# RomanBresson/KAGNN

Measured on AMD Instinct MI355X. Metric: edges/sec KAN-GIN fwd+bwd, hidden=64 grid=5, 1M-node synthetic; HBM % peak, higher is better.
Workload: dtype f32 (fp16 hi/lo split operands, fp32 accumulate)

## Files before the change

kagnn_amd/csrc/aggregate.hip:

```cpp
#include "common.h"
#include "host.h"

namespace kagnn {


__device__ __forceinline__ float4 ld4(const float* p) { return *reinterpret_cast<const float4*>(p); }
__device__ __forceinline__ void fma4(float4& a, float w, const float4& v) {
    a.x = fmaf(w, v.x, a.x); a.y = fmaf(w, v.y, a.y); a.z = fmaf(w, v.z, a.z); a.w = fmaf(w, v.w, a.w);
}

__device__ __forceinline__ float edge_w(const AggArgs& a, int e, int j, long i) {
    float w = a.ew ? a.ew[e] : 1.0f;
    if (a.in_scale) w *= a.in_scale[j];
    if (a.skip_self && j == (int)i) w = 0.0f;
    return w;
}

__device__ __forceinline__ void stats_products(const AggArgs& a, long row, int c4, const float4& o, float4& pa, float4& pb) {
    const float4 y = ld4(a.st_y + row * a.st_ldy + c4), m = ld4(a.st_mean + c4), q = ld4(a.st_rstd + c4);
    pa = o;
    pb = make_float4(o.x * ((y.x - m.x) * q.x), o.y * ((y.y - m.y) * q.y), o.z * ((y.z - m.z) * q.z), o.w * ((y.w - m.w) * q.w));
}

template <int LPR, bool STATS = false>
__global__ __launch_bounds__(256) void agg_rows_v4_kernel(AggArgs a) {
    const unsigned wg = (blockIdx.x & 7) * (gridDim.x >> 3) + (blockIdx.x >> 3);
    const long gid = (wg * 256L + threadIdx.x) / LPR;
    const int c4 = (threadIdx.x % LPR) * 4;
    const bool live = gid < a.N && c4 < a.F;
    if (!STATS && !live) return;
    float4 pa = make_float4(0.f, 0.f, 0.f, 0.f), pb = pa;
    if (live) {
        const int s = a.rowptr[gid], t = a.rowptr[gid + 1];
        const bool hub = (t - s) > a.hub_threshold;
        float4 acc = ld4(a.x + gid * a.ldx + c4);
        const float sw = a.self_scale * (a.in_scale ? a.in_scale[gid] : 1.0f);
        acc.x *= sw; acc.y *= sw; acc.z *= sw; acc.w *= sw;
        if (!hub) {
            int e = s;
            for (; e + 4 <= t; e += 4) {
                const int j0 = a.col[e], j1 = a.col[e + 1], j2 = a.col[e + 2], j3 = a.col[e + 3];
                const float4 v0 = ld4(a.x + (long)j0 * a.ldx + c4);
                const float4 v1 = ld4(a.x + (long)j1 * a.ldx + c4);
                const float4 v2 = ld4(a.x + (long)j2 * a.ldx + c4);
                const float4 v3 = ld4(a.x + (long)j3 * a.ldx + c4);
                fma4(acc, edge_w(a, e, j0, gid), v0);
                fma4(acc, edge_w(a, e + 1, j1, gid), v1);
                fma4(acc, edge_w(a, e + 2, j2, gid), v2);
                fma4(acc, edge_w(a, e + 3, j3, gid), v3);
            }
            for (; e < t; ++e) {
                const int j = a.col[e];
                fma4(acc, edge_w(a, e, j, gid), ld4(a.x + (long)j * a.ldx + c4));
            }
        }
        const float os = a.out_scale ? a.out_scale[gid] : 1.0f;
        float4 b = make_float4(0.f, 0.f, 0.f, 0.f);
        if (a.bias) b = ld4(a.bias + c4);
        float4 o = make_float4(fmaf(os, acc.x, b.x), fmaf(os, acc.y, b.y), fmaf(os, acc.z, b.z), fmaf(os, acc.w, b.w));
        if (a.col_scale) {
            const float4 cs = ld4(a.col_scale + c4), ch = ld4(a.col_shift + c4);
            const float cnt = (float)(t - s) + a.self_scale;
            o.x = fmaf(cs.x, o.x, cnt * ch.x); o.y = fmaf(cs.y, o.y, cnt * ch.y);
            o.z = fmaf(cs.z, o.z, cnt * ch.z); o.w = fmaf(cs.w, o.w, cnt * ch.w);
        }
        if (a.addend && !hub) {
            const float4 d = ld4(a.addend + gid * a.lda + c4);
            o.x += d.x; o.y += d.y; o.z += d.z; o.w += d.w;
        }
        *reinterpret_cast<float4*>(a.out + gid * a.ldo + c4) = o;
        if (STATS && !hub) stats_products(a, gid, c4, o, pa, pb);
    }
    if constexpr (STATS) {
        __shared__ float4 s_a[256], s_b[256];
        s_a[threadIdx.x] = pa; s_b[threadIdx.x] = pb;
        __syncthreads();
        if (threadIdx.x < LPR && c4 < a.F && wg * 256L < a.N * LPR) {
            constexpr int R = 256 / LPR;
#pragma unroll 4
            for (int k = 1; k < R; ++k) {
                const float4 u = s_a[k * LPR + threadIdx.x], v = s_b[k * LPR + threadIdx.x];
                pa.x += u.x; pa.y += u.y; pa.z += u.z; pa.w += u.w;
                pb.x += v.x; pb.y += v.y; pb.z += v.z; pb.w += v.w;
            }
            *reinterpret_cast<float4*>(a.st_partial + (wg * 2L + 0) * a.F + c4) = pa;
            *reinterpret_cast<float4*>(a.st_partial + (wg * 2L + 1) * a.F + c4) = pb;
        }
    }
}

template <int LPR>
__global__ __launch_bounds__(256) void agg_rows_ep_kernel(AggArgs a) {
    constexpr int EP = 16 / LPR;
    const long gid = (blockIdx.x * 256L + threadIdx.x) >> 4;
    const int l16 = threadIdx.x & 15, cg = l16 % LPR, eg = l16 / LPR;
    const int c4 = cg * 4;
    const bool live = gid < a.N && c4 < a.F;
    const long row = min(gid, a.N - 1);
    const int cc = live ? c4 : 0;
    const int s = a.rowptr[row], t = a.rowptr[row + 1];
    const bool hub = (t - s) > a.hub_threshold;
    float4 acc = make_float4(0.f, 0.f, 0.f, 0.f);
    if (!hub) {
        int e = s + eg;
        for (; e + EP < t; e += 2 * EP) {
            const int j0 = a.col[e], j1 = a.col[e + EP];
            const float4 v0 = ld4(a.x + (long)j0 * a.ldx + cc);
            const float4 v1 = ld4(a.x + (long)j1 * a.ldx + cc);
            fma4(acc, edge_w(a, e, j0, row), v0);
            fma4(acc, edge_w(a, e + EP, j1, row), v1);
        }
        if (e < t) {
            const int j = a.col[e];
            fma4(acc, edge_w(a, e, j, row), ld4(a.x + (long)j * a.ldx + cc));
        }
    }
#pragma unroll
    for (int o = LPR; o < 16; o <<= 1) {
        acc.x += __shfl_xor(acc.x, o); acc.y += __shfl_xor(acc.y, o);
        acc.z += __shfl_xor(acc.z, o); acc.w += __shfl_xor(acc.w, o);
    }
    if (live && eg == 0) {
        const float sw = a.self_scale * (a.in_scale ? a.in_scale[row] : 1.0f);
        const float4 xs = ld4(a.x + row * a.ldx + c4);
        const float os = a.out_scale ? a.out_scale[row] : 1.0f;
        float4 b = make_float4(0.f, 0.f, 0.f, 0.f);
        if (a.bias) b = ld4(a.bias + c4);
        float4 o = make_float4(fmaf(os, fmaf(sw, xs.x, acc.x), b.x), fmaf(os, fmaf(sw, xs.y, acc.y), b.y),
                               fmaf(os, fmaf(sw, xs.z, acc.z), b.z), fmaf(os, fmaf(sw, xs.w, acc.w), b.w));
        if (a.col_scale) {
            const float4 cs = ld4(a.col_scale + c4), ch = ld4(a.col_shift + c4);
            const float cnt = (float)(t - s) + a.self_scale;
            o.x = fmaf(cs.x, o.x, cnt * ch.x); o.y = fmaf(cs.y, o.y, cnt * ch.y);
            o.z = fmaf(cs.z, o.z, cnt * ch.z); o.w = fmaf(cs.w, o.w, cnt * ch.w);
        }
        if (a.addend && !hub) {
            const float4 d = ld4(a.addend + row * a.lda + c4);
            o.x += d.x; o.y += d.y; o.z += d.z; o.w += d.w;
        }
        *reinterpret_cast<float4*>(a.out + row * a.ldo + c4) = o;
    }
}

template <int LPR>
__global__ __launch_bounds__(256) void agg_hub_v4_kernel(AggArgs a, const int* __restrict__ seg,
                                                         float* __restrict__ part, int ldp) {
    __shared__ float4 s_part[256];
    const int row = seg[3 * blockIdx.x], e0 = seg[3 * blockIdx.x + 1], e1 = seg[3 * blockIdx.x + 2];
    constexpr int G = 256 / LPR;
    const int g = threadIdx.x / LPR, lg = threadIdx.x % LPR, c4 = lg * 4;
    float4 acc = make_float4(0.f, 0.f, 0.f, 0.f);
    if (c4 < a.F) {
        int e = e0 + g;
        for (; e + 3 * G < e1; e += 4 * G) {
            const int j0 = a.col[e], j1 = a.col[e + G], j2 = a.col[e + 2 * G], j3 = a.col[e + 3 * G];
            const float4 v0 = ld4(a.x + (long)j0 * a.ldx + c4);
            const float4 v1 = ld4(a.x + (long)j1 * a.ldx + c4);
            const float4 v2 = ld4(a.x + (long)j2 * a.ldx + c4);
            const float4 v3 = ld4(a.x + (long)j3 * a.ldx + c4);
            fma4(acc, edge_w(a, e, j0, row), v0);
            fma4(acc, edge_w(a, e + G, j1, row), v1);
            fma4(acc, edge_w(a, e + 2 * G, j2, row), v2);
            fma4(acc, edge_w(a, e + 3 * G, j3, row), v3);
        }
        for (; e < e1; e += G) {
            const int j = a.col[e];
            fma4(acc, edge_w(a, e, j, row), ld4(a.x + (long)j * a.ldx + c4));
        }
    }
    s_part[threadIdx.x] = acc;
    __syncthreads();
    if (g == 0 && c4 < a.F) {
#pragma unroll 8
// ... 229 lines not shown
        }
        for (; b < b1; ++b) a += partial[b * per + k];
    }
    s_part[sub][e] = a;
    __syncthreads();
    if (sub == 0 && k < per) {
        float t = s_part[0][e];
#pragma unroll
        for (int q = 1; q < 8; ++q) t += s_part[q][e];
        g_table[k] = t;
    }
}

int embedding_fwd(const int64_t* idx, long stride, long N, const float* table, int V, int F, float* out, long ldo, int accumulate,
                  hipStream_t st) {
    if (N == 0) return KAGNN_OK;
    embedding_fwd_kernel<<<cdiv(N, 4), 256, 0, st>>>(idx, stride, N, table, V, F, out, ldo, accumulate);
    KAGNN_LAUNCH_CHECK();
    return KAGNN_OK;
}

size_t embedding_bwd_ws_bytes(long N, int V, int F) { return (size_t)cdiv(max(N, 1L), kEmbRows) * V * F * sizeof(float); }

int embedding_bwd(const int64_t* idx, long stride, long N, const float* g, long ldg, int V, int F, float* g_table, float* ws,
                  size_t ws_bytes, hipStream_t st) {
    if (V == 0) return KAGNN_OK;
    if (V > 512) return fail(KAGNN_ERR_UNSUPPORTED, "%s: tables of at most 512 rows (the categorical encoders of the graph-level models)", "embedding_bwd");
    if (ws_bytes < embedding_bwd_ws_bytes(N, V, F)) return fail(KAGNN_ERR_ARG, "%s: workspace too small", "embedding_bwd");
    const size_t tbl = (size_t)V * 64 * sizeof(float);
    const int waves = 4 * tbl <= 64 * 1024 ? 4 : 2 * tbl <= 128 * 1024 ? 2 : 1;
    const int nb = cdiv(max(N, 1L), (long)kEmbRows);
    const size_t lds = waves * tbl;
    if (lds > 64 * 1024) {
        static unsigned long long configured = 0;
        if (auto first_use_ = first_use_on_this_device(configured)) {
            KAGNN_HIP(hipFuncSetAttribute((const void*)embedding_bwd_partial_kernel<1>, hipFuncAttributeMaxDynamicSharedMemorySize, 128 * 1024 + 1024));
            KAGNN_HIP(hipFuncSetAttribute((const void*)embedding_bwd_partial_kernel<2>, hipFuncAttributeMaxDynamicSharedMemorySize, 128 * 1024 + 1024));
        }
    }
    const dim3 grid((unsigned)nb, (unsigned)cdiv(F, 64));
    if (waves == 4) embedding_bwd_partial_kernel<4><<<grid, 256, lds, st>>>(idx, stride, N, g, ldg, V, F, ws);
    else if (waves == 2) embedding_bwd_partial_kernel<2><<<grid, 128, lds, st>>>(idx, stride, N, g, ldg, V, F, ws);
    else embedding_bwd_partial_kernel<1><<<grid, 64, lds, st>>>(idx, stride, N, g, ldg, V, F, ws);
    KAGNN_LAUNCH_CHECK();
    embedding_bwd_reduce_kernel<<<cdiv((long)V * F, 32), 256, 0, st>>>(ws, nb, V, F, g_table);
    KAGNN_LAUNCH_CHECK();
    return KAGNN_OK;
}

static bool vec4_ok(const AggArgs& a) {
    auto al = [](const void* p) { return (reinterpret_cast<uintptr_t>(p) & 15) == 0; };
    return a.F % 4 == 0 && a.F <= 256 && a.ldx % 4 == 0 && a.ldo % 4 == 0 && al(a.x) && al(a.out) &&
           (!a.bias || al(a.bias)) && (!a.addend || (al(a.addend) && a.lda % 4 == 0)) &&
           (!a.col_scale || (al(a.col_scale) && al(a.col_shift)));
}

size_t aggregate_ws_bytes(long num_hub_seg, int F) { return (size_t)num_hub_seg * (size_t)((F + 3) & ~3) * sizeof(float); }

int aggregate_hub_rows(const AggArgs& a, const int* hub_seg, long num_hub_seg, float* ws, size_t ws_bytes, hipStream_t st) {
    if (num_hub_seg <= 0) return KAGNN_OK;
    const int ldp = (a.F + 3) & ~3;
    if ((size_t)num_hub_seg * ldp * sizeof(float) > ws_bytes) return fail(KAGNN_ERR_ARG, "%s: workspace too small", "aggregate_hub_rows");
#define HUBS(LPR)                                                                                   \
    {                                                                                               \
        agg_hub_v4_kernel<LPR><<<(unsigned)num_hub_seg, 256, 0, st>>>(a, hub_seg, ws, ldp);         \
        KAGNN_LAUNCH_CHECK();                                                                       \
        agg_hub_merge_kernel<LPR><<<(unsigned)num_hub_seg, 256, 0, st>>>(a, hub_seg, num_hub_seg, ws, ldp); \
        KAGNN_LAUNCH_CHECK();                                                                       \
    }
    if (a.F <= 4) HUBS(1) else if (a.F <= 8) HUBS(2) else if (a.F <= 16) HUBS(4) else if (a.F <= 32) HUBS(8)
    else if (a.F <= 64) HUBS(16) else if (a.F <= 128) HUBS(32) else HUBS(64)
#undef HUBS
    return KAGNN_OK;
}

static int stats_lpr(int F) { return F <= 32 ? 8 : F <= 64 ? 16 : F <= 128 ? 32 : 64; }
bool aggregate_stats_ok(const AggArgs& a) {
    auto al = [](const void* p) { return (reinterpret_cast<uintptr_t>(p) & 15) == 0; };
    return vec4_ok(a) && a.F > 16 && a.st_y && a.st_mean && a.st_rstd && a.st_partial && a.st_ldy % 4 == 0 && al(a.st_y) &&
           al(a.st_mean) && al(a.st_rstd) && al(a.st_partial);
}
long aggregate_stats_rows(long N, int F, long num_hub_seg) { return (long)cdiv(N * stats_lpr(F), 256) + (num_hub_seg > 0 ? num_hub_seg : 0); }

int aggregate_sum(const AggArgs& a, const int* hub_seg, long num_hub_seg, float* ws, size_t ws_bytes, hipStream_t st) {
    if (a.N == 0) return KAGNN_OK;
    const bool stats = a.st_partial != nullptr;
    if (stats && !aggregate_stats_ok(a)) return fail(KAGNN_ERR_UNSUPPORTED, "%s: column statistics need 16-byte aligned fp32 rows of 17..256 columns", "aggregate_sum");
    if (!vec4_ok(a)) {
        AggArgs b = a;
        b.hub_threshold = 0x7fffffff;
        dim3 grid((unsigned)a.N, cdiv(a.F, 256));
        agg_rows_generic_kernel<<<grid, 256, 0, st>>>(b);
        KAGNN_LAUNCH_CHECK();
        return KAGNN_OK;
    }
    AggArgs b = a;
    if (num_hub_seg == 0 || hub_seg == nullptr) b.hub_threshold = 0x7fffffff;
    const int ldp = (a.F + 3) & ~3;
    if (b.hub_threshold != 0x7fffffff && (ws == nullptr || ws_bytes < aggregate_ws_bytes(num_hub_seg, a.F)))
        return fail(KAGNN_ERR_ARG, "%s: workspace too small for the hub segments (see kagnn_aggregate_workspace_bytes)", "aggregate_sum");
#define HUBS(LPR, ST)                                                                               \
    if (b.hub_threshold != 0x7fffffff) {                                                            \
        agg_hub_v4_kernel<LPR><<<(unsigned)num_hub_seg, 256, 0, st>>>(b, hub_seg, ws, ldp);         \
        KAGNN_LAUNCH_CHECK();                                                                       \
        agg_hub_merge_kernel<LPR, ST><<<(unsigned)num_hub_seg, 256, 0, st>>>(b, hub_seg, num_hub_seg, ws, ldp, (long)cdiv(a.N * LPR, 256)); \
        KAGNN_LAUNCH_CHECK();                                                                       \
    }
#define AGG_ROWS_GRID(threads) (cdiv(cdiv((threads), 256), 8) * 8)
#define ROWS(LPR)                                                                     \
    {                                                                                 \
        if (stats) {                                                                  \
            agg_rows_v4_kernel<LPR, true><<<AGG_ROWS_GRID(a.N * LPR), 256, 0, st>>>(b);   \
            KAGNN_LAUNCH_CHECK();                                                     \
            HUBS(LPR, true)                                                           \
        } else {                                                                      \
            agg_rows_v4_kernel<LPR><<<AGG_ROWS_GRID(a.N * LPR), 256, 0, st>>>(b);       \
            KAGNN_LAUNCH_CHECK();                                                     \
            HUBS(LPR, false)                                                          \
        }                                                                             \
    }
#define ROWS_EP(LPR)                                                                  \
    {                                                                                 \
        agg_rows_ep_kernel<LPR><<<cdiv(a.N * 16, 256), 256, 0, st>>>(b);              \
        KAGNN_LAUNCH_CHECK();                                                         \
        HUBS(LPR, false)                                                              \
    }
    if (a.F <= 4) ROWS_EP(1) else if (a.F <= 8) ROWS_EP(2) else if (a.F <= 16) ROWS_EP(4) else if (a.F <= 32) ROWS(8)
    else if (a.F <= 64) ROWS(16)
    else if (a.F <= 128) ROWS(32) else ROWS(64)
#undef ROWS
#undef AGG_ROWS_GRID
#undef ROWS_EP
#undef HUBS
    return KAGNN_OK;
}

int gcn_deg_inv_sqrt(const int* rowptr, const int* col, long N, float* dis, hipStream_t st) {
    if (N == 0) return KAGNN_OK;
    gcn_deg_kernel<<<cdiv(N, 256), 256, 0, st>>>(rowptr, col, N, dis);
    KAGNN_LAUNCH_CHECK();
    return KAGNN_OK;
}

int gine_fwd(const float* x, long ldx, const float* ea, long lde, float* out, long ldo,
             const int* rowptr, const int* col, const int* perm, long N, int F, float self_scale,
             hipStream_t st) {
    if (N == 0) return KAGNN_OK;
    gine_fwd_kernel<<<cdiv(N, 4), 256, 0, st>>>(x, ldx, ea, lde, out, ldo, rowptr, col, perm, N, F, self_scale);
    KAGNN_LAUNCH_CHECK();
    return KAGNN_OK;
}

int gine_bwd(const float* x, long ldx, const float* ea, long lde, const float* gout, long ldg,
             float* gx, long ldgx, float* gea, long ldge, const int* rowptr, const int* col,
             const int* perm, long N, int F, float self_scale, hipStream_t st, int gea_accumulate) {
    if (N == 0) return KAGNN_OK;
    gine_bwd_kernel<<<cdiv(N, 4), 256, 0, st>>>(x, ldx, ea, lde, gout, ldg, gx, ldgx, gea, ldge, rowptr, col, perm, N, F, self_scale, gea_accumulate);
    KAGNN_LAUNCH_CHECK();
    return KAGNN_OK;
}

int segment_pool(const float* x, long ldx, float* out, long ldo, const int* seg, long B, int F,
                 int mean, hipStream_t st) {
    if (B == 0) return KAGNN_OK;
    segment_pool_kernel<<<cdiv(B, 4), 256, 0, st>>>(x, ldx, out, ldo, seg, B, F, mean);
    KAGNN_LAUNCH_CHECK();
    return KAGNN_OK;
}

int segment_bcast(const float* g, long ldg, float* gx, long ldgx, const int* seg, long B, int F,
                  int mean, hipStream_t st) {
    if (B == 0) return KAGNN_OK;
    segment_bcast_kernel<<<cdiv(B, 4), 256, 0, st>>>(g, ldg, gx, ldgx, seg, B, F, mean);
    KAGNN_LAUNCH_CHECK();
    return KAGNN_OK;
}

}
```

kagnn_amd/csrc/common.h:

```cpp
#pragma once
#include <hip/hip_runtime.h>
#include <stdint.h>
#include <stdio.h>
#include <string.h>
#include "../../include/kagnn_hip.h"

namespace kagnn {

extern thread_local char g_err[512];
extern thread_local bool g_half_products;
inline int fail(int code, const char* fmt, const char* a = "", long b = 0, long c = 0) {
    snprintf(g_err, sizeof(g_err), fmt, a, b, c);
    return code;
}
#define KAGNN_CHECK_ARG_AS(fn, cond, msg)                                                \
    do {                                                                                 \
        if (!(cond)) return kagnn::fail(KAGNN_ERR_ARG, "%s: argument check failed: " msg, fn); \
    } while (0)
#define KAGNN_CHECK_ARG(cond, msg) KAGNN_CHECK_ARG_AS(__func__, cond, msg)
#define KAGNN_HIP(...)                                                                   \
    do {                                                                                 \
        hipError_t e_ = (__VA_ARGS__);                                                   \
        if (e_ != hipSuccess) {                                                          \
            snprintf(kagnn::g_err, sizeof(kagnn::g_err), "%s: HIP error at line %d -> %s", __func__, __LINE__, \
// ... 116 lines not shown
    const bool finite = fabsf(x) <= 3.4028234e38f;
    const float nanv = __builtin_nanf("");
#pragma unroll
    for (int r = 0; r <= K; ++r) {
        N[r] = finite ? (inside ? n[r] : 0.0f) : nanv;
        if (DERIV) dN[r] = finite ? (inside ? dN[r] : 0.0f) : nanv;
    }
    return m;
}

template <int K, bool DERIV>
__device__ __forceinline__ int bspline_generic(float x, const float* __restrict__ t ,
                                               int nknots, float (&N)[K + 1], float (&dN)[K + 1]) {
    int cnt = 0;
    for (int j = 0; j < nknots; ++j) cnt += (x >= t[j]) ? 1 : 0;
    const bool inside = cnt >= 1 && cnt < nknots;
    const int m = min(max(cnt - 1, 0), nknots - 2);
    float w[2 * K + 2];
#pragma unroll
    for (int q = 0; q < 2 * K + 2; ++q) w[q] = t[min(max(m - K + q, 0), nknots - 1)];
    float n[K + 1], prev[K + 1];
    n[0] = 1.0f;
#pragma unroll
    for (int r = 1; r <= K; ++r) n[r] = 0.0f;
#pragma unroll
    for (int p = 1; p <= K; ++p) {
#pragma unroll
        for (int r = 0; r <= K; ++r) prev[r] = n[r];
#pragma unroll
        for (int r = 0; r <= p; ++r) {
            const int q0 = K - p + r;
            const float a = (r >= 1) ? (x - w[q0]) / (w[q0 + p] - w[q0]) * prev[r - 1] : 0.0f;
            const float b = (r <= p - 1) ? (w[q0 + p + 1] - x) / (w[q0 + p + 1] - w[q0 + 1]) * prev[r] : 0.0f;
            n[r] = a + b;
        }
        if (DERIV && p == K) {
#pragma unroll
            for (int r = 0; r <= K; ++r) {
                const float lo = (r >= 1) ? prev[r - 1] / (w[r + K] - w[r]) : 0.0f;
                const float hi = (r <= K - 1) ? prev[r] / (w[r + K + 1] - w[r + 1]) : 0.0f;
                dN[r] = (float)K * (lo - hi);
            }
        }
    }
    const bool finite = fabsf(x) <= 3.4028234e38f;
    const float nanv = __builtin_nanf("");
#pragma unroll
    for (int r = 0; r <= K; ++r) {
        N[r] = finite ? (inside ? n[r] : 0.0f) : nanv;
        if (DERIV) dN[r] = finite ? (inside ? dN[r] : 0.0f) : nanv;
    }
    return m;
}

template <int K, bool DERIV, bool PF>
__device__ __forceinline__ int eval_basis(float x, const float* s_knots, const SplineGeom& g,
                                          const float* __restrict__ knots_g, int f, float (&N)[K + 1],
                                          float (&dN)[K + 1]) {
    if constexpr (PF) return bspline_generic<K, DERIV>(x, knots_g + (long)f * g.nknots, g.nknots, N, dN);
    else return bspline_local<K, DERIV>(x, s_knots, g, N, dN);
}

template <int K>
__device__ __forceinline__ float pick_basis(const float (&N)[K + 1], int m, int c) {
    const int d = c - (m - K);
    float a = 0.0f;
#pragma unroll
    for (int r = 0; r <= K; ++r) a = (d == r) ? N[r] : a;
    return a;
}

struct AggArgs {
    const float* x; long ldx;
    float* out; long ldo;
    const int* rowptr; const int* col; const float* ew;
    long N; int F;
    float self_scale;
    const float* in_scale; const float* out_scale; const float* bias;
    int skip_self; int hub_threshold;
    const float* addend; long lda;
    const float* col_scale = nullptr; const float* col_shift = nullptr;
    const float* st_y = nullptr; long st_ldy = 0; const float* st_mean = nullptr; const float* st_rstd = nullptr;
    float* st_partial = nullptr;
};

struct EdgeGradArgs {
    const float* x; long ldx;
    const float* gout; long ldg;
    const int* rowptr; const int* col; const int* perm;
    long N; long E; int F;
    const float* in_scale; const float* out_scale;
    int skip_self; int hub_threshold;
    float* out;
};

struct BnBack {
    const float* y; long ldy;
    const float* tab; int ldt;
    float* gy_out; long ldo;
};
#ifdef __HIPCC__
__device__ __forceinline__ float bn_bwd_value(float g, float y, float m, float A, float B, float C) {
    return __builtin_fmaf(A, g, __builtin_fmaf(B, __fsub_rn(y, m), C));
}
__device__ __forceinline__ void bn_bwd_consts(float q , float gamma, float sum_g, float sum_gxhat, float inv_n, float& A,
                                              float& B, float& C) {
    const float k = __fmul_rn(q, gamma);
    A = k;
    B = -__fmul_rn(__fmul_rn(k, q), __fmul_rn(sum_gxhat, inv_n));
    C = -__fmul_rn(k, __fmul_rn(sum_g, inv_n));
}
#endif

inline hipStream_t as_stream(void* s) { return reinterpret_cast<hipStream_t>(s); }

}
```

kagnn_amd/csrc/fused_calls.hip:

```cpp
#include "host.h"

using namespace kagnn;

namespace {
struct GraphSide {
    const int32_t* rowptr; const int32_t* col; const int32_t* hub_seg; int64_t num_hub_seg; int32_t hub_threshold; float self_scale;
};
struct KanChain {
    int64_t N; int32_t L; const int32_t* widths;
    const float* const* bw; const float* const* sw; const float* const* sc;
    const float* const* acts; const void* const* pack_fwd; const void* const* pack_dx;
    const float* knots; int32_t G, K, mode;
};
struct LayerIn {
    const void* x; int32_t x_dtype; int64_t ldx; const float* in_col_scale; const float* in_col_shift; float* col_mean; float* col_m2;
};
struct LayerGrads {
    const float* gy; int64_t ldgy; void* gx; int32_t gx_dtype; int64_t ldgx; int32_t bf16_gather; const float* gx_addend; int64_t ld_addend;
    float* const* g_bw; float* const* g_sw; float* const* g_sc;
};

struct GineStage {
    const float* x; int64_t ldx; const float* ea; int64_t lde; const int32_t* perm;
    float* g_ea; int64_t ldge;
    int accumulate_g_ea = 0;
    int prepacked = 0;
};
struct BnStage { const float* y; int64_t ldy; const float* weight; const float* mean; const float* rstd; float* g_weight; float* g_bias; };
struct StatsOut { const float* y; int64_t ldy; const float* mean; const float* rstd; float* sums; };
struct DwPiece { unsigned char* base; DwDefer* defer; };

struct LayerLayout {
    size_t fwd_hub_bytes, fwd_scratch, fwd_scratch_bytes, fwd_fix, fwd_fix_bytes, fwd_total;
    size_t bwd_hub_bytes, dw, dw_bytes, g[2], bwd_total;
    size_t bn, bn_ws_bytes, bn_tab, bn_bytes, stats, stats_bytes, bwd_total_all;
    size_t dw_piece[8], dw_piece_bytes[8], dw_pieces_bytes;
    int wmax;
};

void layer_layout_optional(LayerLayout& y, int64_t N, int out, int f0, int64_t num_hub_seg_t) {
    y.bn = y.bwd_total;
    y.bn_ws_bytes = out ? bn_ws_bytes(N, out) : 0;
    y.bn_tab = y.bn + al256z(y.bn_ws_bytes);
    y.bn_bytes = out ? al256z(y.bn_ws_bytes) + al256z(4 * (size_t)((out + 63) & ~63) * sizeof(float)) : 0;
    y.stats = y.bn + y.bn_bytes;
    y.stats_bytes = f0 ? al256z(bn_stats_fold_bytes(aggregate_stats_rows(N, f0, num_hub_seg_t), f0)) : 0;
    y.bwd_total_all = y.stats + y.stats_bytes;
}

int layer_layout(int64_t N, int32_t L, const int32_t* widths, int32_t G, int32_t K, int32_t mode, int64_t num_hub_seg,
                 int64_t num_hub_seg_t, LayerLayout& y) {
    static const char fn[] = "kagnn_gin_kan_layer_workspace_bytes";
    size_t fw = 0, dw = 0;
    y.wmax = 0;
    for (int l = 0; l < L; ++l) {
        int rc = check_kan_dims(fn, widths[l], widths[l + 1], G, K, mode);
        if (rc) return rc;
        size_t b = 0;
        rc = (l == L - 1 ? kagnn_kan_fwd_moments_workspace_bytes : kagnn_kan_fwd_workspace_bytes)(N, widths[l], widths[l + 1], G, K, mode, &b);
        if (rc) return rc;
        fw = b > fw ? b : fw;
        rc = kagnn_kan_bwd_weight_workspace_bytes(N, widths[l], widths[l + 1], G, K, mode, &b); if (rc) return rc;
        dw = b > dw ? b : dw;
        y.dw_piece_bytes[l] = al256z(b);
        y.wmax = widths[l] > y.wmax ? widths[l] : y.wmax;
    }
    y.dw_pieces_bytes = 0;
    for (int l = L - 1; l >= 0; --l) { y.dw_piece[l] = y.dw_pieces_bytes; y.dw_pieces_bytes += y.dw_piece_bytes[l]; }
    y.fwd_hub_bytes = al256z(aggregate_bf16_ws_bytes(num_hub_seg, widths[0]));
    y.fwd_scratch = y.fwd_hub_bytes;
    y.fwd_fix = y.fwd_scratch + al256z(fw);
    y.fwd_total = y.fwd_fix + al256z(widths[0] <= 32 ? kan_sparse_fwd_agg_ws_bytes(num_hub_seg, widths[0], widths[1]) : 0) + 256;
    y.fwd_scratch_bytes = y.fwd_total - y.fwd_scratch;
    y.fwd_fix_bytes = y.fwd_total - y.fwd_fix;
    y.bwd_hub_bytes = al256z(aggregate_bf16_ws_bytes(num_hub_seg_t, widths[0]));
    y.dw = y.bwd_hub_bytes;
    y.dw_bytes = al256z(dw);
    const size_t g_bytes = al256z((size_t)N * y.wmax * sizeof(float));
    y.g[0] = y.dw + y.dw_bytes;
    y.g[1] = y.g[0] + g_bytes;
    y.bwd_total = y.g[1] + g_bytes + 256;
    layer_layout_optional(y, N, 0, 0, 0);
    return KAGNN_OK;
}

int layer_fwd_impl(const GraphSide& gr, const KanChain& c, const LayerIn& in, const GineStage* gine, void* workspace,
                   size_t workspace_bytes, void* stream, const char* fn) {
    (void)fn;
    const int64_t N = c.N;
    const int32_t L = c.L, G = c.G, K = c.K, mode = c.mode;
    const int32_t* widths = c.widths;
    float* const* acts = const_cast<float* const*>(c.acts);
    void* const* pack_fwd = const_cast<void* const*>(c.pack_fwd);
    void* const* pack_dx = const_cast<void* const*>(c.pack_dx);
    KAGNN_CHECK_ARG(N >= 0 && L >= 1 && L <= 8 && widths && c.bw && c.sw && acts && pack_fwd && pack_dx, "bad argument");
    KAGNN_CHECK_ARG((in.in_col_scale == nullptr) == (in.in_col_shift == nullptr), "in_col_scale and in_col_shift must both be given or both be null");
    KAGNN_CHECK_ARG(!in.in_col_scale || in.x_dtype == KAGNN_DTYPE_F32, "the column affine of the gathered matrix needs fp32 rows");
    KAGNN_CHECK_ARG((in.col_mean == nullptr) == (in.col_m2 == nullptr), "col_mean and col_m2 must both be given or both be null");
    LayerLayout lay;
    int rc = layer_layout(N, L, widths, G, K, mode, gr.num_hub_seg, 0, lay);
    if (rc) return rc;
    KAGNN_CHECK_ARG(workspace && workspace_bytes >= lay.fwd_total, "workspace too small (kagnn_gin_kan_layer_workspace_bytes)");
    if (N == 0) return KAGNN_OK;
    unsigned char* ws = static_cast<unsigned char*>(workspace);
    const char* fuse_e = getenv("KAGNN_FUSE_AGG");
    const bool fuse_env = fuse_e != nullptr && atoi(fuse_e) != 0;
    const bool fuse = fuse_env && !gine && !in.in_col_scale && in.x_dtype == KAGNN_DTYPE_F32 && mode == KAGNN_PREC_SPLIT && !(L == 1 && in.col_mean) &&
                      use_sparse_fwd(widths[0], widths[1], G, K, mode) &&
                      kan_sparse_fwd_agg_ok(static_cast<const float*>(in.x), in.ldx, N, widths[0], widths[1], G, K);
    if (gine)
        rc = kagnn_aggregate_gine(static_cast<const float*>(in.x), in.ldx, gine->ea, gine->lde, acts[0], widths[0], gr.rowptr, gr.col, gine->perm, N,
                                  widths[0], gr.self_scale, stream);
    else if (fuse)
        rc = KAGNN_OK;
    else if (in.x_dtype == KAGNN_DTYPE_BF16)
        rc = kagnn_aggregate_sum_bf16(in.x, in.ldx, acts[0], widths[0], KAGNN_DTYPE_F32, gr.rowptr, gr.col, nullptr, N, widths[0], gr.self_scale,
                                      nullptr, nullptr, nullptr, 0, gr.hub_seg, gr.num_hub_seg, gr.hub_threshold, ws, lay.fwd_hub_bytes, stream);
    else if (in.in_col_scale)
        rc = kagnn_aggregate_sum_affine(static_cast<const float*>(in.x), in.ldx, acts[0], widths[0], gr.rowptr, gr.col, N, widths[0], gr.self_scale,
                                        in.in_col_scale, in.in_col_shift, gr.hub_seg, gr.num_hub_seg, gr.hub_threshold, nullptr, 0, ws,
                                        lay.fwd_hub_bytes, stream);
    else
        rc = kagnn_aggregate_sum(static_cast<const float*>(in.x), in.ldx, acts[0], widths[0], gr.rowptr, gr.col, nullptr, N, widths[0],
                                 gr.self_scale, nullptr, nullptr, nullptr, 0, gr.hub_seg, gr.num_hub_seg, gr.hub_threshold, ws, lay.fwd_hub_bytes,
                                 stream);
    if (rc) return rc;
    const bool prepacked = gine && gine->prepacked;
    bool batched = L >= 2 && !prepacked;
    int in_[8], out_[8];
    for (int l = 0; l < L; ++l) {
        in_[l] = widths[l]; out_[l] = widths[l + 1];
        batched = batched && use_split_dx(in_[l], out_[l], G, K, mode) && use_sparse_fwd(in_[l], out_[l], G, K, mode) &&
                  kan_fused_pack_ok(in_[l], out_[l], G + K);
    }
    if (batched) {
        rc = kagnn_kan_pack_batch(L, c.bw, c.sw, c.sc, in_, out_, G, K, mode, pack_fwd, pack_dx, stream);
        if (rc) return rc;
    } else if (!prepacked) {
        for (int l = 0; l < L; ++l) {
            rc = kagnn_kan_pack(c.bw[l], c.sw[l], c.sc ? c.sc[l] : nullptr, in_[l], out_[l], G, K, mode, pack_fwd[l], pack_dx[l], stream);
            if (rc) return rc;
        }
    }
    for (int l = 0; l < L; ++l) {
        if (l == 0 && fuse) {
            KAGNN_STAGE_AS("kagnn_kan_linear_fwd+aggregate_sum (one kernel)", stream);
            rc = kan_sparse_fwd_agg(static_cast<const float*>(in.x), in.ldx, N, gr.rowptr, gr.col, gr.hub_seg, gr.num_hub_seg, gr.hub_threshold,
                                    gr.self_scale, c.knots, in_[0], out_[0], G, K, pack_fwd[0], acts[0], in_[0], acts[1], out_[0],
                                    ws + lay.fwd_fix, lay.fwd_fix_bytes, as_stream(stream));
            if (rc) return rc;
            continue;
        }
        if (l == L - 1 && in.col_mean)
            rc = kagnn_kan_linear_fwd_moments(acts[l], in_[l], N, c.knots, in_[l], out_[l], G, K, mode, pack_fwd[l], acts[l + 1],
                                              out_[l], in.col_mean, in.col_m2, ws + lay.fwd_scratch, lay.fwd_scratch_bytes, stream);
        else
            rc = kagnn_kan_linear_fwd(acts[l], in_[l], N, c.knots, in_[l], out_[l], G, K, mode, pack_fwd[l], acts[l + 1], out_[l],
                                      ws + lay.fwd_scratch, lay.fwd_scratch_bytes, stream);
        if (rc) return rc;
    }
    return KAGNN_OK;
}

int layer_bwd_impl(const GraphSide& gr, const KanChain& c, const LayerGrads& io, const BnStage* bn, const float* bn_sums_in,
                   const StatsOut* so, const GineStage* gine, const DwPiece* piece, void* workspace, size_t workspace_bytes, void* stream,
                   const char* fn) {
    const int64_t N = c.N;
    const int32_t L = c.L, G = c.G, K = c.K, mode = c.mode;
    const int32_t* widths = c.widths;
    const float* const* acts = c.acts;
    void* const gx = io.gx;
    KAGNN_CHECK_ARG(N >= 0 && L >= 1 && L <= 8 && widths && c.sw && acts && c.pack_dx && io.g_sw, "bad argument");
    KAGNN_CHECK_ARG(!io.gx_addend || (gx && io.gx_dtype == KAGNN_DTYPE_F32 && !io.bf16_gather && io.ld_addend >= widths[0]),
                    "gx_addend needs an fp32 gx and fp32 gather operands");
    LayerLayout lay;
    int rc = layer_layout(N, L, widths, G, K, mode, 0, gr.num_hub_seg, lay);
    if (rc) return rc;
    layer_layout_optional(lay, N, bn ? widths[L] : 0, so ? widths[0] : 0, gr.num_hub_seg);
    KAGNN_CHECK_ARG(!so || (so->y && so->mean && so->rstd && so->sums && so->ldy >= widths[0] && gx && io.gx_dtype == KAGNN_DTYPE_F32 && !io.bf16_gather),
                    "the previous norm's statistics need its input, mean, rstd and an fp32 gx");
    KAGNN_CHECK_ARG(!bn_sums_in || bn, "bn_sums belongs to the BatchNorm stage");
    if (!(workspace && workspace_bytes >= lay.bwd_total_all))
        return fail(KAGNN_ERR_ARG, bn ? "%s: workspace too small (kagnn_gin_kan_layer_workspace_bytes + kagnn_gin_kan_layer_bwd_bn_workspace_bytes)"
                                      : "%s: workspace too small (kagnn_gin_kan_layer_workspace_bytes)", fn);
    if (N == 0) return KAGNN_OK;
    unsigned char* ws = static_cast<unsigned char*>(workspace);
    const int wmax = lay.wmax;
    unsigned char* gbuf[2] = {ws + lay.g[0], ws + lay.g[1]};
    auto dw = [&](int l, const float* g, long ldg) {
        unsigned char* area = piece ? piece->base + lay.dw_piece[l] : ws + lay.dw;
        const size_t bytes = piece ? lay.dw_piece_bytes[l] : lay.dw_bytes;
        return kan_linear_bwd_weight(acts[l], widths[l], nullptr, g, ldg, N, c.knots, widths[l], widths[l + 1], G, K, mode, c.sw[l],
                                     c.sc ? c.sc[l] : nullptr, io.g_bw ? io.g_bw[l] : nullptr, io.g_sw[l], io.g_sc ? io.g_sc[l] : nullptr,
                                     area, bytes, stream, piece ? piece->defer : nullptr);
    };
    const float* g = io.gy;
    long ldg = io.ldgy;
    int cur = 0;
    bool gh0_bf16 = false;
    bool bn_in_dx = false;
    BnBack bnb{};
    if (bn) {
        const int out = widths[L], ldt = (out + 63) & ~63;
        KAGNN_CHECK_ARG(bn->y && bn->mean && bn->rstd && bn->ldy >= out && N >= 2, "bad BatchNorm stage");
        unsigned char* bws = ws + lay.bn;
        float* tab = reinterpret_cast<float*>(ws + lay.bn_tab);
        bnb = BnBack{bn->y, (long)bn->ldy, tab, ldt, reinterpret_cast<float*>(gbuf[1]), (long)out};
        const int in = widths[L - 1];
        bn_in_dx = mode == KAGNN_PREC_SPLIT && use_split_dx(in, out, G, K, mode) && out <= wmax && !(L == 1 && (gx == nullptr || io.bf16_gather)) &&
                   fits32(N, ldg) && kan_split_dx_bn_ok(ldg, in, out, G, K, bnb, g);
        if (bn_in_dx && bn_sums_in) {
            KAGNN_STAGE_AS("kagnn_batchnorm_bwd statistics given (in ..._layer_bwd_bn)", stream);
            rc = bn_bwd_stats_given(bn_sums_in, N, out, bn->weight, bn->mean, bn->rstd, bn->g_weight, bn->g_bias, tab, ldt, as_stream(stream));
            if (rc) return rc;
        } else if (bn_in_dx) {
            KAGNN_STAGE_AS("kagnn_batchnorm_bwd statistics (in ..._layer_bwd_bn)", stream);
            rc = bn_bwd_stats(bn->y, bn->ldy, g, ldg, N, out, bn->weight, bn->mean, bn->rstd, bn->g_weight, bn->g_bias, tab, ldt, bws,
                              lay.bn_ws_bytes, as_stream(stream));
            if (rc) return rc;
        } else {
            if (out > wmax) return fail(KAGNN_ERR_UNSUPPORTED, "%s: a BatchNorm stage wider than every layer input is not covered", fn);
            KAGNN_STAGE_AS("kagnn_batchnorm_bwd", stream);
            rc = bn_bwd(bn->y, bn->ldy, g, ldg, N, out, bn->weight, bn->mean, bn->rstd, 1, 0.0f, 0ULL, reinterpret_cast<float*>(gbuf[1]), out,
                        bn->g_weight, bn->g_bias, bws, lay.bn_ws_bytes, as_stream(stream));
            if (rc) return rc;
            g = reinterpret_cast<const float*>(gbuf[1]); ldg = out;
        }
    }
    for (int l = L - 1; l >= 0; --l) {
        const int in = widths[l], out = widths[l + 1];
        const bool fused_bn = bn_in_dx && l == L - 1;
        if (fused_bn) {
            {
                KAGNN_STAGE_AS("kagnn_kan_linear_bwd_input", stream);
                rc = kan_split_dx_bn(acts[l], in, g, ldg, N, c.knots, in, out, G, K, c.pack_dx[l], reinterpret_cast<float*>(gbuf[0]), in, bnb,
                                     as_stream(stream));
            }
            if (rc) return rc;
            rc = dw(l, bnb.gy_out, bnb.ldo);
            if (rc) return rc;
            if (l == 0 && gx == nullptr) break;
            g = reinterpret_cast<const float*>(gbuf[0]); ldg = in; cur = 1;
            continue;
        }
        rc = dw(l, g, ldg);
        if (rc) return rc;
        if (l == 0 && gx == nullptr) break;
        const bool b16 = l == 0 && io.bf16_gather && mode == KAGNN_PREC_SPLIT && K == 3 && G + K <= 8 && out <= 128 && in % 8 == 0 &&
                         in <= 512  &&
                         use_split_dx(in, out, G, K, mode);
        rc = kagnn_kan_linear_bwd_input(acts[l], in, g, ldg, N, c.knots, in, out, G, K, mode, c.pack_dx[l], gbuf[cur], in,
                                        b16 ? KAGNN_DTYPE_BF16 : KAGNN_DTYPE_F32, stream);
        if (rc) return rc;
        g = reinterpret_cast<const float*>(gbuf[cur]); ldg = in; cur ^= 1;
        gh0_bf16 = b16;
    }
    if (gx == nullptr) return KAGNN_OK;
    const int f0 = widths[0];
    if (gine)
        return gine_bwd(gine->x, gine->ldx, gine->ea, gine->lde, g, ldg, static_cast<float*>(gx), io.ldgx, gine->g_ea, gine->ldge,
                        gr.rowptr, gr.col, gine->perm, N, f0, gr.self_scale, as_stream(stream), gine->accumulate_g_ea);
    if (gh0_bf16 || io.gx_dtype == KAGNN_DTYPE_BF16) {
        const void* src = g;
        if (!gh0_bf16) {
            rc = kagnn_rows_to_bf16(g, ldg, gbuf[cur], f0, N, f0, stream);
            if (rc) return rc;
            src = gbuf[cur];
        }
        return kagnn_aggregate_sum_bf16(src, f0, gx, io.ldgx, io.gx_dtype, gr.rowptr, gr.col, nullptr, N, f0, gr.self_scale, nullptr, nullptr,
                                        nullptr, 0, gr.hub_seg, gr.num_hub_seg, gr.hub_threshold, ws, lay.bwd_hub_bytes, stream);
    }
    if (so) {
        AggArgs a{g, ldg, static_cast<float*>(gx), io.ldgx, gr.rowptr, gr.col, nullptr, N, f0, gr.self_scale, nullptr, nullptr, nullptr,
                  0, gr.hub_threshold > 0 ? gr.hub_threshold : 0x7fffffff, io.gx_addend, io.ld_addend};
        float* partial = reinterpret_cast<float*>(ws + lay.stats);
        a.st_y = so->y; a.st_ldy = so->ldy; a.st_mean = so->mean; a.st_rstd = so->rstd; a.st_partial = partial;
        KAGNN_CHECK_ARG(ldg >= f0 && io.ldgx >= f0 && (!io.gx_addend || io.ld_addend >= f0), "leading dimension smaller than num_feat");
        if (!aggregate_stats_ok(a)) return fail(KAGNN_ERR_UNSUPPORTED, "%s: the previous norm's statistics need 17..256 input features in 16-byte aligned fp32 rows", fn);
        {
            KAGNN_STAGE_AS("kagnn_aggregate_sum", stream);
            rc = aggregate_sum(a, gr.hub_seg, gr.num_hub_seg, reinterpret_cast<float*>(ws), lay.bwd_hub_bytes, as_stream(stream));
            if (rc) return rc;
        }
        KAGNN_STAGE_AS("kagnn_batchnorm_bwd statistics fold", stream);
        const bool hubs = gr.num_hub_seg > 0 && gr.hub_seg != nullptr && gr.hub_threshold > 0;
        return bn_sums_from_partials(partial, aggregate_stats_rows(N, f0, hubs ? gr.num_hub_seg : 0), f0, so->sums, as_stream(stream));
    }
    return kagnn_aggregate_sum_add(g, ldg, static_cast<float*>(gx), io.ldgx, gr.rowptr, gr.col, nullptr, N, f0, gr.self_scale, nullptr,
                                   nullptr, nullptr, 0, gr.hub_seg, gr.num_hub_seg, gr.hub_threshold, io.gx_addend, io.ld_addend, ws,
                                   lay.bwd_hub_bytes, stream);
}

struct StackLayout {
    LayerLayout layer;
    size_t fwd_layer_bytes, bn_ws, bn_ws_bytes, moments, fwd_total;
    size_t bwd_layer_bytes, pp[2], arena, arena_conv_bytes, arena_bytes, bwd_total;
};

int stack_layout(int64_t N, int32_t nconv, int32_t L, const int32_t* widths, int32_t G, int32_t K, int32_t mode, StackLayout& s) {
    int rc = layer_layout(N, L, widths, G, K, mode, 0, 0, s.layer);
    if (rc) return rc;
    layer_layout_optional(s.layer, N, widths[L], 0, 0);
    s.fwd_layer_bytes = al256z(s.layer.fwd_total);
    s.bn_ws = s.fwd_layer_bytes;
    s.bn_ws_bytes = bn_ws_bytes(N, widths[L]);
    s.moments = s.bn_ws + al256z(s.bn_ws_bytes);
    s.fwd_total = s.moments + al256z(2 * (size_t)widths[L] * sizeof(float)) + 256;
    s.bwd_layer_bytes = al256z(s.layer.bwd_total_all);
    const size_t g_bytes = al256z((size_t)N * widths[0] * sizeof(float));
    s.pp[0] = s.bwd_layer_bytes;
    s.pp[1] = s.pp[0] + g_bytes;
    s.arena = s.pp[1] + g_bytes;
    s.arena_conv_bytes = nconv * L <= kDwDeferMax ? s.layer.dw_pieces_bytes : 0;
    s.arena_bytes = s.arena_conv_bytes * (size_t)nconv;
    s.bwd_total = s.arena + s.arena_bytes + 256;
    return KAGNN_OK;
}

int stack_fwd_impl(const float* x, int64_t ldx, const float* edge_attr, int64_t lde, int64_t N, const int32_t* rowptr,
                   const int32_t* col, const int32_t* perm, const float* self_scale, int32_t nconv,
                   int32_t L, const int32_t* widths, const float* const* bw, const float* const* sw,
                   const float* const* sc, const float* knots, int32_t G, int32_t K, int32_t mode,
                   float* const* acts, void* const* pack_fwd, void* const* pack_dx,
                   const float* const* bn_weight, const float* const* bn_bias, float* const* running_mean,
                   float* const* running_var, const float* momentum, const float* eps,
                   float* const* h, float* const* save_mean, float* const* save_rstd,
                   void* workspace, size_t workspace_bytes, void* stream, bool prepacked) {
    static const char fn[] = "kagnn_gine_kan_stack_fwd";
    ModeScope mode_scope_(mode);
    KAGNN_CHECK_ARG_AS(fn, nconv >= 1 && L >= 1 && L <= 8 && widths && self_scale && bw && sw && acts && pack_fwd && pack_dx && bn_weight && bn_bias &&
                       momentum && eps && h && save_mean && save_rstd, "null array");
    KAGNN_CHECK_ARG_AS(fn, widths[0] == widths[L] && N >= 2, "hidden -> hidden chains, at least two rows (batch statistics)");
    StackLayout lay;
    int rc = stack_layout(N, nconv, L, widths, G, K, mode, lay);
    if (rc) return rc;
    KAGNN_CHECK_ARG_AS(fn, workspace && workspace_bytes >= lay.fwd_total, "workspace too small (kagnn_gine_kan_stack_workspace_bytes)");
    unsigned char* ws = static_cast<unsigned char*>(workspace);
    float* mom = reinterpret_cast<float*>(ws + lay.moments);
    const int H = widths[L];
    int in_[16], out_[16];
    bool batch = nconv * L <= 16;
// ... 574 lines not shown
```

kagnn_amd/csrc/host.h:

```cpp
#pragma once
#include "common.h"

namespace kagnn {

struct RbfArgs;

size_t aggregate_ws_bytes(long num_hub_seg, int F);
int aggregate_sum(const AggArgs& a, const int* hub_seg, long num_hub_seg, float* ws, size_t ws_bytes, hipStream_t st);
bool aggregate_stats_ok(const AggArgs& a);
long aggregate_stats_rows(long N, int F, long num_hub_seg);
int gcn_deg_inv_sqrt(const int* rowptr, const int* col, long N, float* dis, hipStream_t st);
int gine_fwd(const float* x, long ldx, const float* ea, long lde, float* out, long ldo, const int* rowptr, const int* col, const
             int* perm, long N, int F, float self_scale, hipStream_t st);
int gine_bwd(const float* x, long ldx, const float* ea, long lde, const float* gout, long ldg, float* gx, long ldgx, float* gea,
             long ldge, const int* rowptr, const int* col, const int* perm, long N, int F, float self_scale, hipStream_t st, int
             gea_accumulate = 0);
int segment_pool(const float* x, long ldx, float* out, long ldo, const int* seg, long B, int F, int mean, hipStream_t st);
int segment_bcast(const float* g, long ldg, float* gx, long ldgx, const int* seg, long B, int F, int mean, hipStream_t st);
int embedding_fwd(const int64_t* idx, long stride, long N, const float* table, int V, int F, float* out, long ldo, int accumulate,
                  hipStream_t st);
int embedding_bwd(const int64_t* idx, long stride, long N, const float* g, long ldg, int V, int F, float* g_table, float* ws, size_t
                  ws_bytes, hipStream_t st);
size_t embedding_bwd_ws_bytes(long N, int V, int F);

int aggregate_hub_rows(const AggArgs& a, const int* hub_seg, long num_hub_seg, float* ws, size_t ws_bytes, hipStream_t st);

int aggregate_edge_grad(const EdgeGradArgs& a, const int* hub_seg, long num_hub_seg, hipStream_t st);

size_t aggregate_bf16_ws_bytes(long num_hub_seg, int F);
bool aggregate_bf16_ok(const void* x, long ldx, const void* out, long ldo, int out_bf16, int F, const float* bias);
int aggregate_sum_bf16(const void* x, long ldx, void* out, long ldo, int out_bf16, const int* rowptr, const int* col, const float*
                       ew, long N, int F, float self_scale, const float* in_scale, const float* out_scale, const float* bias, int
                       skip_self, const int* hub_seg, long num_hub_seg, int hub_threshold, float* ws, size_t ws_bytes, hipStream_t
                       st);
int rows_to_bf16(const float* x, long ldx, void* y, long ldy, long N, int F, hipStream_t st);

bool kan_sparse_fwd_agg_ok(const float* x, long ldx, long N, int in, int out, int G, int K);
size_t kan_sparse_fwd_agg_ws_bytes(long num_hub_seg, int in, int out);
int kan_sparse_fwd_agg(const float* x, long ldx, long N, const int* rowptr, const int* col, const int* hub_seg, long num_hub_seg,
                       int hub_threshold, float self_scale, const float* knots, int in, int out, int G, int K, const void* pack,
                       float* h0, long ldh, float* y, long ldy, void* ws, size_t ws_bytes, hipStream_t st);
bool kan_sparse_fwd_ok(int in, int out, int G, int K);
bool kan_fused_pack_ok(int in, int out, int C);
int kan_fused_pack(const float* bw, const float* sw, const float* sc, int in, int out, int C, void* pack_fwd, void* pack_dx,
                   hipStream_t st);
int kan_fused_pack_batch(int n, const float* const* bw, const float* const* sw, const float* const* sc, const int* in, const int*
                         out, int C, void* const* pack_fwd, void* const* pack_dx, hipStream_t st);
size_t kan_sparse_pack_fwd_bytes(int in, int out, int C);
int kan_sparse_pack_fwd(const float* bw, const float* sw, const float* sc, int in, int out, int C, void* pack_fwd, hipStream_t st);
size_t kan_sparse_fwd_ws_bytes(long N, int in, int out, int C);
int kan_sparse_fwd(const float* x, long ldx, long N, const float* knots, int in, int out, int G, int K, const void* pack, float* y,
                   long ldy, void* ws, size_t ws_bytes, float* col_mean, float* col_m2, hipStream_t st);
bool kan_sparse_fwd_parts_ok(const int* widths, int nparts, int in, int out, int G, int K);
int kan_sparse_fwd_parts(const float* const* parts, const int* widths, const long* lds, int nparts, long N, const float* knots, int
                         in, int out, int G, int K, const void* pack, float* y, long ldy, void* ws, size_t ws_bytes, hipStream_t st,
                         const float* const* part_affine);
bool kan_sparse_fwd_moments_ok(long N, int in, int out, int G, int K);
size_t kan_sparse_fwd_moments_ws_bytes(long N, int out);

size_t bn_stats_fold_bytes(long B, int F);
int bn_sums_from_partials(float* ws, long B, int F, float* sums, hipStream_t st);
int bn_finish_partials(const float* partial, long B, int F, float* sums, hipStream_t st);
int bn_bwd_stats_given(const float* sums, long N, int F, const float* gamma, const float* save_mean, const float* save_rstd, float*
                       g_gamma, float* g_beta, float* tab, int ldt, hipStream_t st);
int col_moments(const float* x, long ldx, long N, int F, float* col_mean, float* col_m2, void* ws, size_t ws_bytes, hipStream_t st);
size_t bn_ws_bytes(long N, int F);
int bn_fwd(const float* x, long ldx, long N, int F, const float* gamma, const float* beta, float* running_mean, float* running_var,
           float momentum, float eps, int training, const float* col_mean, const float* col_m2, float dropout_p, unsigned long long
           dropout_seed, float* y, long ldy, float* save_mean, float* save_rstd, void* ws, size_t ws_bytes, hipStream_t st);
int bn_bwd(const float* x, long ldx, const float* gy, long ldgy, long N, int F, const float* gamma, const float* save_mean, const
           float* save_rstd, int training, float dropout_p, unsigned long long dropout_seed, float* gx, long ldgx, float* g_gamma,
           float* g_beta, void* ws, size_t ws_bytes, hipStream_t st);
int bn_bwd_stats(const float* x, long ldx, const float* gy, long ldgy, long N, int F, const float* gamma, const float* save_mean,
                 const float* save_rstd, float* g_gamma, float* g_beta, float* tab, int ldt, void* ws, size_t ws_bytes, hipStream_t
                 st);
int bn_stats_affine(const float* col_mean, const float* col_m2, long N, int F, const float* gamma, const float* beta, float*
                    running_mean, float* running_var, float momentum, float eps, float* save_mean, float* save_rstd, float* affine,
                    hipStream_t st);
int moments_finish(const float* partial, int P, int F, float* col_mean, float* col_m2, hipStream_t st);

int csr_workspace_bytes(long E, long N, size_t* bytes);
int csr_build(const int64_t* key, const int64_t* val, long E, long N, int* rowptr, int* col, int* perm, int T, int* hub_seg, long
              cap, int64_t* nseg_host, void* ws, size_t ws_bytes, hipStream_t st);
bool csr_small_ok(long E, long N);
size_t csr_small_workspace_bytes(long E);
int csr_build_small(const int64_t* src, const int64_t* dst, long E, long N, int* rowptr, int* col, int* perm, int* rowptr_t, int*
                    col_t, int* perm_t, int* flags, void* ws, size_t ws_bytes, hipStream_t st);

size_t kan_f32_pack_fwd_bytes(int in, int out, int C);
size_t kan_f32_pack_dx_bytes(int in, int out, int C);
int kan_f32_pack(const float* bw, const float* sw, const float* sc, int in, int out, int C, float* pf, float* pd, hipStream_t st);
// ... 217 lines not shown
```

Measured before the change: 4.303 billion.

## Overlap weight-gradient kernels with backward aggregation on a side stream

In layer backward, the weight-gradient kernels for the first layer (and the last layer when there is no BN) are deferred and issued on a per-device side stream. They then run concurrently with the final input-gradient aggregation. The aggregation is split into a head launch that reserves extra LDS to cap its occupancy and leave room for the side-stream kernels, and a tail launch that waits on the side stream's completion event. A lean kernel variant drops the optional scaling and bias fields. This adds a global mutex, extra streams and events, and is disabled under graph capture or via an environment variable.

New measurement: 4.634 billion, median of 6. 7.7% higher.

```diff
diff --git a/kagnn_amd/csrc/aggregate.hip b/kagnn_amd/csrc/aggregate.hip
--- a/kagnn_amd/csrc/aggregate.hip
+++ b/kagnn_amd/csrc/aggregate.hip
@@ -22,9 +22,14 @@
     pb = make_float4(o.x * ((y.x - m.x) * q.x), o.y * ((y.y - m.y) * q.y), o.z * ((y.z - m.z) * q.z), o.w * ((y.w - m.w) * q.w));
 }
 
-template <int LPR, bool STATS = false>
-__global__ __launch_bounds__(256) void agg_rows_v4_kernel(AggArgs a) {
-    const unsigned wg = (blockIdx.x & 7) * (gridDim.x >> 3) + (blockIdx.x >> 3);
+template <int LPR, bool STATS, bool LEAN>
+__device__ __forceinline__ void agg_rows_v4_body(const AggArgs& args) {
+    AggArgs a = args;
+    if constexpr (LEAN) {
+        a.ew = nullptr; a.in_scale = nullptr; a.out_scale = nullptr; a.bias = nullptr; a.skip_self = 0;
+        a.col_scale = nullptr; a.col_shift = nullptr;
+    }
+    const unsigned wg = (LEAN ? a.wg0 : 0u) + (blockIdx.x & 7) * (gridDim.x >> 3) + (blockIdx.x >> 3);
     const long gid = (wg * 256L + threadIdx.x) / LPR;
     const int c4 = (threadIdx.x % LPR) * 4;
     const bool live = gid < a.N && c4 < a.F;
@@ -89,6 +94,12 @@
     }
 }
 
+template <int LPR, bool STATS = false>
+__global__ __launch_bounds__(256) void agg_rows_v4_kernel(AggArgs a) { agg_rows_v4_body<LPR, STATS, false>(a); }
+
+template <int LPR>
+__global__ __launch_bounds__(256) void agg_rows_v4_corun_kernel(AggArgs a) { agg_rows_v4_body<LPR, false, true>(a); }
+
 template <int LPR>
 __global__ __launch_bounds__(256) void agg_rows_ep_kernel(AggArgs a) {
     constexpr int EP = 16 / LPR;
@@ -484,8 +495,14 @@
 }
 long aggregate_stats_rows(long N, int F, long num_hub_seg) { return (long)cdiv(N * stats_lpr(F), 256) + (num_hub_seg > 0 ? num_hub_seg : 0); }
 
-int aggregate_sum(const AggArgs& a, const int* hub_seg, long num_hub_seg, float* ws, size_t ws_bytes, hipStream_t st) {
+bool aggregate_corun_ok(const AggArgs& a) {
+    return vec4_ok(a) && a.F > 32 && a.F <= 64 && !a.ew && !a.in_scale && !a.out_scale && !a.bias && !a.skip_self && !a.col_scale && !a.st_partial;
+}
+
+int aggregate_sum(const AggArgs& a, const int* hub_seg, long num_hub_seg, float* ws, size_t ws_bytes, hipStream_t st, const AggCorun* corun) {
     if (a.N == 0) return KAGNN_OK;
+    if (corun && !(aggregate_corun_ok(a) && corun->head_pct >= 0 && corun->head_pct < 100 && corun->side_done))
+        return fail(KAGNN_ERR_ARG, "%s: the co-run launch does not cover this call", "aggregate_sum");
     const bool stats = a.st_partial != nullptr;
     if (stats && !aggregate_stats_ok(a)) return fail(KAGNN_ERR_UNSUPPORTED, "%s: column statistics need 16-byte aligned fp32 rows of 17..256 columns", "aggregate_sum");
     if (!vec4_ok(a)) {
@@ -516,7 +533,19 @@
             KAGNN_LAUNCH_CHECK();                                                     \
             HUBS(LPR, true)                                                           \
         } else {                                                                      \
-            agg_rows_v4_kernel<LPR><<<AGG_ROWS_GRID(a.N * LPR), 256, 0, st>>>(b);       \
+            if (corun && LPR == 16) {         \
+                const unsigned total = AGG_ROWS_GRID(a.N * LPR);       \
+                const unsigned head = (unsigned)((unsigned long)total * (unsigned)corun->head_pct / 100) & ~7u; \
+                if (head) {                                                           \
+                    agg_rows_v4_corun_kernel<16><<<head, 256, kAggCorunLds, st>>>(b); \
+                    KAGNN_LAUNCH_CHECK();                                             \
+                }                                                                     \
+                KAGNN_HIP(hipStreamWaitEvent(st, corun->side_done, 0));               \
+                AggArgs t = b;                                                        \
+                t.wg0 = head;                                                         \
+                agg_rows_v4_corun_kernel<16><<<total - head, 256, 0, st>>>(t);        \
+            } else                                                                    \
+                agg_rows_v4_kernel<LPR><<<AGG_ROWS_GRID(a.N * LPR), 256, 0, st>>>(b);   \
             KAGNN_LAUNCH_CHECK();                                                     \
             HUBS(LPR, false)                                                          \
         }                                                                             \
diff --git a/kagnn_amd/csrc/common.h b/kagnn_amd/csrc/common.h
--- a/kagnn_amd/csrc/common.h
+++ b/kagnn_amd/csrc/common.h
@@ -222,6 +222,7 @@
     const float* col_scale = nullptr; const float* col_shift = nullptr;
     const float* st_y = nullptr; long st_ldy = 0; const float* st_mean = nullptr; const float* st_rstd = nullptr;
     float* st_partial = nullptr;
+    unsigned wg0 = 0;
 };
 
 struct EdgeGradArgs {
diff --git a/kagnn_amd/csrc/fused_calls.hip b/kagnn_amd/csrc/fused_calls.hip
--- a/kagnn_amd/csrc/fused_calls.hip
+++ b/kagnn_amd/csrc/fused_calls.hip
@@ -1,4 +1,5 @@
 #include "host.h"
+#include <mutex>
 
 using namespace kagnn;
 
@@ -162,6 +163,61 @@
     return KAGNN_OK;
 }
 
+struct BwdSide { hipStream_t stream = nullptr; hipEvent_t fork = nullptr, join = nullptr; };
+constexpr int kBwdSideMaxDevices = 64;
+std::mutex g_bwd_side_mu;
+BwdSide g_bwd_side[kBwdSideMaxDevices];
+
+class BwdFork {
+    std::unique_lock<std::mutex> lk_;
+    BwdSide* s_ = nullptr;
+    hipStream_t caller_ = nullptr;
+    bool forked_ = false, recorded_ = false;
+public:
+    BwdFork() = default;
+    BwdFork(const BwdFork&) = delete;
+    BwdFork& operator=(const BwdFork&) = delete;
+    int prepare(hipStream_t caller) {
+        int dev = 0;
+        KAGNN_HIP(hipGetDevice(&dev));
+        if (dev < 0 || dev >= kBwdSideMaxDevices) return fail(KAGNN_ERR_UNSUPPORTED, "%s: device index out of range", "layer_bwd");
+        lk_ = std::unique_lock<std::mutex>(g_bwd_side_mu);
+        BwdSide& s = g_bwd_side[dev];
+        if (!s.stream) KAGNN_HIP(hipStreamCreateWithFlags(&s.stream, hipStreamNonBlocking));
+        if (!s.fork) KAGNN_HIP(hipEventCreateWithFlags(&s.fork, hipEventDisableTiming));
+        if (!s.join) KAGNN_HIP(hipEventCreateWithFlags(&s.join, hipEventDisableTiming));
+        s_ = &s; caller_ = caller;
+        return KAGNN_OK;
+    }
+    int fork() {
+        KAGNN_HIP(hipEventRecord(s_->fork, caller_));
+        KAGNN_HIP(hipStreamWaitEvent(s_->stream, s_->fork, 0));
+        forked_ = true;
+        return KAGNN_OK;
+    }
+    hipStream_t side() const { return s_->stream; }
+    int side_done(hipEvent_t* ev) {
+        KAGNN_HIP(hipEventRecord(s_->join, s_->stream));
+        recorded_ = true;
+        *ev = s_->join;
+        return KAGNN_OK;
+    }
+    void joined() { forked_ = false; }
+    int join() {
+        if (!forked_) return KAGNN_OK;
+        forked_ = false;
+        if (!recorded_) KAGNN_HIP(hipEventRecord(s_->join, s_->stream));
+        KAGNN_HIP(hipStreamWaitEvent(caller_, s_->join, 0));
+        return KAGNN_OK;
+    }
+    ~BwdFork() { (void)join(); }
+};
+
+constexpr int kAggCorunHeadPct = 35;
+bool dw_corun_ok(int in, int out, int G, int K, int mode) {
+    return use_split_dw(in, out, G, K, mode) && !g_half_products && K == 3 && G + K <= 8 && in > 32 && in <= 64 && out <= 64;
+}
+
 int layer_bwd_impl(const GraphSide& gr, const KanChain& c, const LayerGrads& io, const BnStage* bn, const float* bn_sums_in,
                    const StatsOut* so, const GineStage* gine, const DwPiece* piece, void* workspace, size_t workspace_bytes, void* stream,
                    const char* fn) {
@@ -187,12 +243,39 @@
     unsigned char* ws = static_cast<unsigned char*>(workspace);
     const int wmax = lay.wmax;
     unsigned char* gbuf[2] = {ws + lay.g[0], ws + lay.g[1]};
-    auto dw = [&](int l, const float* g, long ldg) {
+    auto dw_on = [&](void* st, int l, const float* g, long ldg) {
         unsigned char* area = piece ? piece->base + lay.dw_piece[l] : ws + lay.dw;
         const size_t bytes = piece ? lay.dw_piece_bytes[l] : lay.dw_bytes;
         return kan_linear_bwd_weight(acts[l], widths[l], nullptr, g, ldg, N, c.knots, widths[l], widths[l + 1], G, K, mode, c.sw[l],
                                      c.sc ? c.sc[l] : nullptr, io.g_bw ? io.g_bw[l] : nullptr, io.g_sw[l], io.g_sc ? io.g_sc[l] : nullptr,
-                                     area, bytes, stream, piece ? piece->defer : nullptr);
+                                     area, bytes, st, piece ? piece->defer : nullptr);
+    };
+    BwdFork side;
+    struct { int l; const float* g; long ldg; } deferred[2];
+    int n_deferred = 0;
+    bool overlap = false;
+    if (gx && !gine && !piece && !so && !io.bf16_gather && io.gx_dtype == KAGNN_DTYPE_F32 && dw_corun_ok(widths[0], widths[1], G, K, mode)) {
+        const char* env = getenv("KAGNN_BWD_OVERLAP");
+        const AggArgs probe{reinterpret_cast<const float*>(gbuf[0]), widths[0], static_cast<float*>(gx), io.ldgx, gr.rowptr, gr.col, nullptr, N,
+                            widths[0], gr.self_scale, nullptr, nullptr, nullptr, 0, 0x7fffffff, io.gx_addend, io.ld_addend};
+        const bool gx_in_ws = static_cast<unsigned char*>(gx) + (size_t)N * io.ldgx * sizeof(float) > ws &&
+                              static_cast<unsigned char*>(gx) < ws + workspace_bytes;
+        overlap = (env == nullptr || atoi(env) != 0) && io.ldgx >= widths[0] && (!io.gx_addend || io.ld_addend >= widths[0]) && !gx_in_ws &&
+                  aggregate_corun_ok(probe);
+        if (overlap) {
+            hipStreamCaptureStatus cap = hipStreamCaptureStatusNone;
+            if (hipStreamIsCapturing(as_stream(stream), &cap) != hipSuccess) { (void)hipGetLastError(); overlap = false; }
+            else overlap = cap == hipStreamCaptureStatusNone;
+        }
+        if (overlap) { rc = side.prepare(as_stream(stream)); if (rc) return rc; }
+    }
+    auto dw = [&](int l, const float* g, long ldg) {
+        const bool alive = l == 0 || (l == L - 1 && !bn);
+        if (overlap && alive && dw_corun_ok(widths[l], widths[l + 1], G, K, mode)) {
+            deferred[n_deferred++] = {l, g, ldg};
+            return (int)KAGNN_OK;
+        }
+        return dw_on(stream, l, g, ldg);
     };
     const float* g = io.gy;
     long ldg = io.ldgy;
@@ -257,6 +340,24 @@
     }
     if (gx == nullptr) return KAGNN_OK;
     const int f0 = widths[0];
+    if (overlap) {
+        rc = side.fork();
+        if (rc) return rc;
+        for (int k = 0; k < n_deferred; ++k) {
+            rc = dw_on(side.side(), deferred[k].l, deferred[k].g, deferred[k].ldg);
+            if (rc) return rc;
+        }
+        const AggArgs a{g, ldg, static_cast<float*>(gx), io.ldgx, gr.rowptr, gr.col, nullptr, N, f0, gr.self_scale, nullptr, nullptr, nullptr,
+                        0, gr.hub_threshold > 0 ? gr.hub_threshold : 0x7fffffff, io.gx_addend, io.ld_addend};
+        AggCorun corun{kAggCorunHeadPct * n_deferred, nullptr};
+        rc = side.side_done(&corun.side_done);
+        if (rc) return rc;
+        KAGNN_STAGE_AS("kagnn_aggregate_sum", stream);
+        rc = aggregate_sum(a, gr.hub_seg, gr.num_hub_seg, reinterpret_cast<float*>(ws), lay.bwd_hub_bytes, as_stream(stream), &corun);
+        if (rc) return rc;
+        side.joined();
+        return KAGNN_OK;
+    }
     if (gine)
         return gine_bwd(gine->x, gine->ldx, gine->ea, gine->lde, g, ldg, static_cast<float*>(gx), io.ldgx, gine->g_ea, gine->ldge,
                         gr.rowptr, gr.col, gine->perm, N, f0, gr.self_scale, as_stream(stream), gine->accumulate_g_ea);
diff --git a/kagnn_amd/csrc/host.h b/kagnn_amd/csrc/host.h
--- a/kagnn_amd/csrc/host.h
+++ b/kagnn_amd/csrc/host.h
@@ -6,7 +6,12 @@
 struct RbfArgs;
 
 size_t aggregate_ws_bytes(long num_hub_seg, int F);
-int aggregate_sum(const AggArgs& a, const int* hub_seg, long num_hub_seg, float* ws, size_t ws_bytes, hipStream_t st);
+struct AggCorun { int head_pct; hipEvent_t side_done; };
+constexpr unsigned kAggCorunLds = 40000;
+constexpr int kAggCorunVgprs = 40;
+int aggregate_sum(const AggArgs& a, const int* hub_seg, long num_hub_seg, float* ws, size_t ws_bytes, hipStream_t st,
+                  const AggCorun* corun = nullptr);
+bool aggregate_corun_ok(const AggArgs& a);
 bool aggregate_stats_ok(const AggArgs& a);
 long aggregate_stats_rows(long N, int F, long num_hub_seg);
 int gcn_deg_inv_sqrt(const int* rowptr, const int* col, long N, float* dis, hipStream_t st);
```
